# CMU-Perceptual-Computing-Lab/caffe_rtpose

Measured on NVIDIA H100. Metric: frames/sec at 656x368 COCO-18, higher is better.
Workload: dtype f16x2 (2 fp16 planes, 3 wgmma MMAs per MAC, fp32 accumulate)

## Files before the change

### caffe_rtpose_b200/csrc/conv_tc.cu

```cuda
#include <cuda.h>
#include <stdlib.h>
#include <string.h>

#include <algorithm>
#include <atomic>
#include <string>

#include "common.h"
#include "conv_tc.h"
#include "kernels.h"

namespace pe {

struct TcArgs {
    const float* bias;
    __nv_bfloat16* out; int out_pitch, out_coff; long long out_plane;
    float* planar; int planar_C, planar_coff;
    int cout, relu;
    const float* out_scale;
    int ksize, pad, kblocks_per_tap, cin_k;
    int W, H, Wp, Hs;
    long long M;
    int chunk_iters;
    unsigned* range;
};

__device__ __forceinline__ uint32_t smem_u32(const void* p) { return (uint32_t)__cvta_generic_to_shared(p); }

__device__ __forceinline__ void mbar_init(uint64_t* bar, uint32_t count) {
    asm volatile("mbarrier.init.shared::cta.b64 [%0], %1;" ::"r"(smem_u32(bar)), "r"(count));
}
__device__ __forceinline__ void mbar_expect_tx(uint64_t* bar, uint32_t bytes) {
    asm volatile("mbarrier.arrive.expect_tx.shared::cta.b64 _, [%0], %1;" ::"r"(smem_u32(bar)), "r"(bytes) : "memory");
}
__device__ __forceinline__ void mbar_arrive(uint64_t* bar) {
    asm volatile("mbarrier.arrive.shared::cta.b64 _, [%0];" ::"r"(smem_u32(bar)) : "memory");
}
__device__ __forceinline__ void mbar_wait(uint64_t* bar, uint32_t parity) {
    uint32_t done;
    do {
        asm volatile(
            "{\n\t"
            ".reg .pred p;\n\t"
            "mbarrier.try_wait.parity.shared::cta.b64 p, [%1], %2;\n\t"
            "selp.u32 %0, 1, 0, p;\n\t"
            "}" : "=r"(done) : "r"(smem_u32(bar)), "r"(parity) : "memory");
    } while (!done);
}
__device__ __forceinline__ void tma_load_3d(void* dst, const CUtensorMap* map, uint64_t* bar, int c0, int c1, int c2) {
    asm volatile(
        "cp.async.bulk.tensor.3d.shared::cluster.global.tile.mbarrier::complete_tx::bytes [%0], [%1, {%3, %4, %5}], [%2];"
        ::"r"(smem_u32(dst)), "l"(map), "r"(smem_u32(bar)), "r"(c0), "r"(c1), "r"(c2) : "memory");
}

__device__ __forceinline__ void pdl_wait() { asm volatile("griddepcontrol.wait;" ::: "memory"); }
__device__ __forceinline__ void pdl_launch_dependents() { asm volatile("griddepcontrol.launch_dependents;" ::: "memory"); }

__device__ __forceinline__ uint64_t wg_desc(uint32_t saddr) {
    uint64_t d = 0;
    d |= (uint64_t)((saddr >> 4) & 0x3FFF);
    d |= (uint64_t)1 << 16;
    d |= (uint64_t)64 << 32;
    d |= (uint64_t)1 << 62;
    return d;
}
__device__ __forceinline__ void wg_fence() { asm volatile("wgmma.fence.sync.aligned;" ::: "memory"); }
__device__ __forceinline__ void wg_commit() { asm volatile("wgmma.commit_group.sync.aligned;" ::: "memory"); }
__device__ __forceinline__ void wg_wait_all() { asm volatile("wgmma.wait_group.sync.aligned 0;" ::: "memory"); }

template <int N> struct Wgmma;
template <> struct Wgmma<16> {
    template <bool F16> __device__ __forceinline__ static void mma(float* d, uint64_t da, uint64_t db, uint32_t scale_d) {
        if (F16) asm volatile(
            "{\n.reg .pred p;\nsetp.ne.b32 p, %10, 0;\n"
            "wgmma.mma_async.sync.aligned.m64n16k16.f32.f16.f16 {%0,%1,%2,%3,%4,%5,%6,%7}, %8, %9, p, 1, 1, 0, 0;\n}"
            : "+f"(d[0]), "+f"(d[1]), "+f"(d[2]), "+f"(d[3]), "+f"(d[4]), "+f"(d[5]), "+f"(d[6]), "+f"(d[7])
            : "l"(da), "l"(db), "r"(scale_d));
        else asm volatile(
            "{\n.reg .pred p;\nsetp.ne.b32 p, %10, 0;\n"
            "wgmma.mma_async.sync.aligned.m64n16k16.f32.bf16.bf16 {%0,%1,%2,%3,%4,%5,%6,%7}, %8, %9, p, 1, 1, 0, 0;\n}"
            : "+f"(d[0]), "+f"(d[1]), "+f"(d[2]), "+f"(d[3]), "+f"(d[4]), "+f"(d[5]), "+f"(d[6]), "+f"(d[7])
            : "l"(da), "l"(db), "r"(scale_d));
    }
};
template <> struct Wgmma<32> {
    template <bool F16> __device__ __forceinline__ static void mma(float* d, uint64_t da, uint64_t db, uint32_t scale_d) {
        if (F16) asm volatile(
            "{\n.reg .pred p;\nsetp.ne.b32 p, %18, 0;\n"
            "wgmma.mma_async.sync.aligned.m64n32k16.f32.f16.f16 {%0,%1,%2,%3,%4,%5,%6,%7,%8,%9,%10,%11,%12,%13,%14,%15}, %16, %17, p, 1, 1, 0, 0;\n}"
            : "+f"(d[0]), "+f"(d[1]), "+f"(d[2]), "+f"(d[3]), "+f"(d[4]), "+f"(d[5]), "+f"(d[6]), "+f"(d[7]), "+f"(d[8]), "+f"(d[9]), "+f"(d[10]), "+f"(d[11]), "+f"(d[12]), "+f"(d[13]), "+f"(d[14]), "+f"(d[15])
            : "l"(da), "l"(db), "r"(scale_d));
        else asm volatile(
            "{\n.reg .pred p;\nsetp.ne.b32 p, %18, 0;\n"
            "wgmma.mma_async.sync.aligned.m64n32k16.f32.bf16.bf16 {%0,%1,%2,%3,%4,%5,%6,%7,%8,%9,%10,%11,%12,%13,%14,%15}, %16, %17, p, 1, 1, 0, 0;\n}"
            : "+f"(d[0]), "+f"(d[1]), "+f"(d[2]), "+f"(d[3]), "+f"(d[4]), "+f"(d[5]), "+f"(d[6]), "+f"(d[7]), "+f"(d[8]), "+f"(d[9]), "+f"(d[10]), "+f"(d[11]), "+f"(d[12]), "+f"(d[13]), "+f"(d[14]), "+f"(d[15])
            : "l"(da), "l"(db), "r"(scale_d));
    }
};
template <> struct Wgmma<48> {
    template <bool F16> __device__ __forceinline__ static void mma(float* d, uint64_t da, uint64_t db, uint32_t scale_d) {
        if (F16) asm volatile(
            "{\n.reg .pred p;\nsetp.ne.b32 p, %26, 0;\n"
            "wgmma.mma_async.sync.aligned.m64n48k16.f32.f16.f16 {%0,%1,%2,%3,%4,%5,%6,%7,%8,%9,%10,%11,%12,%13,%14,%15,%16,%17,%18,%19,%20,%21,%22,%23}, %24, %25, p, 1, 1, 0, 0;\n}"
            : "+f"(d[0]), "+f"(d[1]), "+f"(d[2]), "+f"(d[3]), "+f"(d[4]), "+f"(d[5]), "+f"(d[6]), "+f"(d[7]), "+f"(d[8]), "+f"(d[9]), "+f"(d[10]), "+f"(d[11]), "+f"(d[12]), "+f"(d[13]), "+f"(d[14]), "+f"(d[15]), "+f"(d[16]), "+f"(d[17]), "+f"(d[18]), "+f"(d[19]), "+f"(d[20]), "+f"(d[21]), "+f"(d[22]), "+f"(d[23])
            : "l"(da), "l"(db), "r"(scale_d));
        else asm volatile(
            "{\n.reg .pred p;\nsetp.ne.b32 p, %26, 0;\n"
            "wgmma.mma_async.sync.aligned.m64n48k16.f32.bf16.bf16 {%0,%1,%2,%3,%4,%5,%6,%7,%8,%9,%10,%11,%12,%13,%14,%15,%16,%17,%18,%19,%20,%21,%22,%23}, %24, %25, p, 1, 1, 0, 0;\n}"
            : "+f"(d[0]), "+f"(d[1]), "+f"(d[2]), "+f"(d[3]), "+f"(d[4]), "+f"(d[5]), "+f"(d[6]), "+f"(d[7]), "+f"(d[8]), "+f"(d[9]), "+f"(d[10]), "+f"(d[11]), "+f"(d[12]), "+f"(d[13]), "+f"(d[14]), "+f"(d[15]), "+f"(d[16]), "+f"(d[17]), "+f"(d[18]), "+f"(d[19]), "+f"(d[20]), "+f"(d[21]), "+f"(d[22]), "+f"(d[23])
            : "l"(da), "l"(db), "r"(scale_d));
    }
};
template <> struct Wgmma<64> {
    template <bool F16> __device__ __forceinline__ static void mma(float* d, uint64_t da, uint64_t db, uint32_t scale_d) {
        if (F16) asm volatile(
            "{\n.reg .pred p;\nsetp.ne.b32 p, %34, 0;\n"
            "wgmma.mma_async.sync.aligned.m64n64k16.f32.f16.f16 {%0,%1,%2,%3,%4,%5,%6,%7,%8,%9,%10,%11,%12,%13,%14,%15,%16,%17,%18,%19,%20,%21,%22,%23,%24,%25,%26,%27,%28,%29,%30,%31}, %32, %33, p, 1, 1, 0, 0;\n}"
            : "+f"(d[0]), "+f"(d[1]), "+f"(d[2]), "+f"(d[3]), "+f"(d[4]), "+f"(d[5]), "+f"(d[6]), "+f"(d[7]), "+f"(d[8]), "+f"(d[9]), "+f"(d[10]), "+f"(d[11]), "+f"(d[12]), "+f"(d[13]), "+f"(d[14]), "+f"(d[15]), "+f"(d[16]), "+f"(d[17]), "+f"(d[18]), "+f"(d[19]), "+f"(d[20]), "+f"(d[21]), "+f"(d[22]), "+f"(d[23]), "+f"(d[24]), "+f"(d[25]), "+f"(d[26]), "+f"(d[27]), "+f"(d[28]), "+f"(d[29]), "+f"(d[30]), "+f"(d[31])
            : "l"(da), "l"(db), "r"(scale_d));
        else asm volatile(
            "{\n.reg .pred p;\nsetp.ne.b32 p, %34, 0;\n"
            "wgmma.mma_async.sync.aligned.m64n64k16.f32.bf16.bf16 {%0,%1,%2,%3,%4,%5,%6,%7,%8,%9,%10,%11,%12,%13,%14,%15,%16,%17,%18,%19,%20,%21,%22,%23,%24,%25,%26,%27,%28,%29,%30,%31}, %32, %33, p, 1, 1, 0, 0;\n}"
            : "+f"(d[0]), "+f"(d[1]), "+f"(d[2]), "+f"(d[3]), "+f"(d[4]), "+f"(d[5]), "+f"(d[6]), "+f"(d[7]), "+f"(d[8]), "+f"(d[9]), "+f"(d[10]), "+f"(d[11]), "+f"(d[12]), "+f"(d[13]), "+f"(d[14]), "+f"(d[15]), "+f"(d[16]), "+f"(d[17]), "+f"(d[18]), "+f"(d[19]), "+f"(d[20]), "+f"(d[21]), "+f"(d[22]), "+f"(d[23]), "+f"(d[24]), "+f"(d[25]), "+f"(d[26]), "+f"(d[27]), "+f"(d[28]), "+f"(d[29]), "+f"(d[30]), "+f"(d[31])
            : "l"(da), "l"(db), "r"(scale_d));
    }
};
template <> struct Wgmma<128> {
    template <bool F16> __device__ __forceinline__ static void mma(float* d, uint64_t da, uint64_t db, uint32_t scale_d) {
        if (F16) asm volatile(
            "{\n.reg .pred p;\nsetp.ne.b32 p, %66, 0;\n"
            "wgmma.mma_async.sync.aligned.m64n128k16.f32.f16.f16 {%0,%1,%2,%3,%4,%5,%6,%7,%8,%9,%10,%11,%12,%13,%14,%15,%16,%17,%18,%19,%20,%21,%22,%23,%24,%25,%26,%27,%28,%29,%30,%31,%32,%33,%34,%35,%36,%37,%38,%39,%40,%41,%42,%43,%44,%45,%46,%47,%48,%49,%50,%51,%52,%53,%54,%55,%56,%57,%58,%59,%60,%61,%62,%63}, %64, %65, p, 1, 1, 0, 0;\n}"
            : "+f"(d[0]), "+f"(d[1]), "+f"(d[2]), "+f"(d[3]), "+f"(d[4]), "+f"(d[5]), "+f"(d[6]), "+f"(d[7]), "+f"(d[8]), "+f"(d[9]), "+f"(d[10]), "+f"(d[11]), "+f"(d[12]), "+f"(d[13]), "+f"(d[14]), "+f"(d[15]), "+f"(d[16]), "+f"(d[17]), "+f"(d[18]), "+f"(d[19]), "+f"(d[20]), "+f"(d[21]), "+f"(d[22]), "+f"(d[23]), "+f"(d[24]), "+f"(d[25]), "+f"(d[26]), "+f"(d[27]), "+f"(d[28]), "+f"(d[29]), "+f"(d[30]), "+f"(d[31]), "+f"(d[32]), "+f"(d[33]), "+f"(d[34]), "+f"(d[35]), "+f"(d[36]), "+f"(d[37]), "+f"(d[38]), "+f"(d[39]), "+f"(d[40]), "+f"(d[41]), "+f"(d[42]), "+f"(d[43]), "+f"(d[44]), "+f"(d[45]), "+f"(d[46]), "+f"(d[47]), "+f"(d[48]), "+f"(d[49]), "+f"(d[50]), "+f"(d[51]), "+f"(d[52]), "+f"(d[53]), "+f"(d[54]), "+f"(d[55]), "+f"(d[56]), "+f"(d[57]), "+f"(d[58]), "+f"(d[59]), "+f"(d[60]), "+f"(d[61]), "+f"(d[62]), "+f"(d[63])
            : "l"(da), "l"(db), "r"(scale_d));
        else asm volatile(
            "{\n.reg .pred p;\nsetp.ne.b32 p, %66, 0;\n"
            "wgmma.mma_async.sync.aligned.m64n128k16.f32.bf16.bf16 {%0,%1,%2,%3,%4,%5,%6,%7,%8,%9,%10,%11,%12,%13,%14,%15,%16,%17,%18,%19,%20,%21,%22,%23,%24,%25,%26,%27,%28,%29,%30,%31,%32,%33,%34,%35,%36,%37,%38,%39,%40,%41,%42,%43,%44,%45,%46,%47,%48,%49,%50,%51,%52,%53,%54,%55,%56,%57,%58,%59,%60,%61,%62,%63}, %64, %65, p, 1, 1, 0, 0;\n}"
            : "+f"(d[0]), "+f"(d[1]), "+f"(d[2]), "+f"(d[3]), "+f"(d[4]), "+f"(d[5]), "+f"(d[6]), "+f"(d[7]), "+f"(d[8]), "+f"(d[9]), "+f"(d[10]), "+f"(d[11]), "+f"(d[12]), "+f"(d[13]), "+f"(d[14]), "+f"(d[15]), "+f"(d[16]), "+f"(d[17]), "+f"(d[18]), "+f"(d[19]), "+f"(d[20]), "+f"(d[21]), "+f"(d[22]), "+f"(d[23]), "+f"(d[24]), "+f"(d[25]), "+f"(d[26]), "+f"(d[27]), "+f"(d[28]), "+f"(d[29]), "+f"(d[30]), "+f"(d[31]), "+f"(d[32]), "+f"(d[33]), "+f"(d[34]), "+f"(d[35]), "+f"(d[36]), "+f"(d[37]), "+f"(d[38]), "+f"(d[39]), "+f"(d[40]), "+f"(d[41]), "+f"(d[42]), "+f"(d[43]), "+f"(d[44]), "+f"(d[45]), "+f"(d[46]), "+f"(d[47]), "+f"(d[48]), "+f"(d[49]), "+f"(d[50]), "+f"(d[51]), "+f"(d[52]), "+f"(d[53]), "+f"(d[54]), "+f"(d[55]), "+f"(d[56]), "+f"(d[57]), "+f"(d[58]), "+f"(d[59]), "+f"(d[60]), "+f"(d[61]), "+f"(d[62]), "+f"(d[63])
            : "l"(da), "l"(db), "r"(scale_d));
    }
};

__device__ __forceinline__ void range_publish(unsigned* range, float m) {
    if (!range) return;
#pragma unroll
    for (int o = 16; o > 0; o >>= 1) m = fmaxf(m, __shfl_xor_sync(0xffffffffu, m, o));
    if ((threadIdx.x & 31) == 0 && m > 0.f) atomicMax(range, __float_as_uint(m));
}

constexpr int TC_BM = 128;
constexpr int TC_BK = 64;
constexpr int TC_WROWS = TC_BM + 8;
constexpr int TC_KMAX = TC_WROWS - TC_BM + 1;
constexpr int TC_THREADS = 384;
constexpr int TC_PRODUCER_REGS = 40, TC_CONSUMER_REGS = 232;
constexpr int TC_SMEM_BUDGET = 220 * 1024;

__host__ __device__ constexpr int tc_window_rows(int ksize) { return ksize == 1 ? TC_BM : TC_WROWS; }

template <int BN, int PLANES> struct TcShape {
    static constexpr int A_BYTES = PLANES * TC_WROWS * 128;
    static constexpr int B_PLANE = BN * 128;
    static constexpr int B_BYTES = PLANES * B_PLANE;
    static constexpr int W_STAGES = 3 * A_BYTES + 6 * B_BYTES <= TC_SMEM_BUDGET ? 3 : 2;
    static constexpr int B_FIT = (TC_SMEM_BUDGET - W_STAGES * A_BYTES) / B_BYTES;
    static constexpr int B_STAGES = B_FIT > 8 ? 8 : B_FIT;
    static constexpr int SMEM = W_STAGES * A_BYTES + B_STAGES * B_BYTES + 1024;
};

template <int BN, int PLANES>
__global__ void __launch_bounds__(TC_THREADS, 1)
conv_wg_kernel(const __grid_constant__ CUtensorMap tmA, const __grid_constant__ CUtensorMap tmB, const TcArgs a) {
    using S = TcShape<BN, PLANES>;
    constexpr int WS = S::W_STAGES, BS = S::B_STAGES;
    constexpr bool F16 = planes_are_fp16(PLANES);
    constexpr int NACC = BN / 2;
    static_assert(S::B_STAGES >= 2, "shared memory holds fewer than two weight tiles");

    extern __shared__ uint8_t smem_raw[];
    uint8_t* smem = (uint8_t*)(((uintptr_t)smem_raw + 1023) & ~(uintptr_t)1023);
    uint8_t* const wring = smem;
    uint8_t* const bring = smem + WS * S::A_BYTES;
    __shared__ __align__(8) uint64_t wfull[WS], wempty[WS], bfull[BS], bempty[BS];
    __shared__ float s_bias[BN];

    const int warp = threadIdx.x >> 5, lane = threadIdx.x & 31;
    const long long m0 = (long long)blockIdx.x * TC_BM;
    const int n0 = blockIdx.y * BN;
    const int ks = a.ksize, taps = ks * ks;
    const int num_k = taps * a.kblocks_per_tap;

    if (threadIdx.x == 0) {
        for (int s = 0; s < WS; s++) { mbar_init(&wfull[s], 1); mbar_init(&wempty[s], 8); }
        for (int s = 0; s < BS; s++) { mbar_init(&bfull[s], 1); mbar_init(&bempty[s], 8); }
        asm volatile("fence.mbarrier_init.release.cluster;" ::: "memory");
        asm volatile("prefetch.tensormap [%0];" ::"l"(&tmA) : "memory");
        asm volatile("prefetch.tensormap [%0];" ::"l"(&tmB) : "memory");
    }
    for (int i = threadIdx.x; i < BN; i += TC_THREADS) s_bias[i] = (n0 + i < a.cout) ? a.bias[n0 + i] : 0.f;
    __syncthreads();
    pdl_launch_dependents();
    pdl_wait();

    if (warp < 4) {
        asm volatile("setmaxnreg.dec.sync.aligned.u32 %0;" ::"n"(TC_PRODUCER_REGS));
        if (threadIdx.x == 0) {
            const uint32_t a_tx = PLANES * tc_window_rows(ks) * 128;
            int wc = 0, bc = 0;
            for (int kb = 0; kb < a.kblocks_per_tap; kb++)
                for (int r = 0; r < ks; r++, wc++) {
                    const int w = wc % WS;
                    mbar_wait(&wempty[w], ((uint32_t)(wc / WS) & 1u) ^ 1u);
                    mbar_expect_tx(&wfull[w], a_tx);
                    const int row0 = (int)(m0 + (long long)(r - a.pad) * a.Wp - a.pad);
                    tma_load_3d(wring + (size_t)w * S::A_BYTES, &tmA, &wfull[w], kb * TC_BK, row0, 0);
                    for (int q = 0; q < ks; q++, bc++) {
                        const int b = bc % BS;
                        mbar_wait(&bempty[b], ((uint32_t)(bc / BS) & 1u) ^ 1u);
                        mbar_expect_tx(&bfull[b], S::B_BYTES);
                        tma_load_3d(bring + (size_t)b * S::B_BYTES, &tmB, &bfull[b], (r * ks + q) * a.cin_k + kb * TC_BK, n0, 0);
                    }
                }
        }
        return;
    }
    asm volatile("setmaxnreg.inc.sync.aligned.u32 %0;" ::"n"(TC_CONSUMER_REGS));

    const int wg = (warp >> 2) - 1;
    float acc_h[NACC], sum_h[NACC], acc_c[NACC];
#pragma unroll
    for (int j = 0; j < NACC; j++) { acc_h[j] = 0.f; sum_h[j] = 0.f; acc_c[j] = 0.f; }
    const int cs = a.chunk_iters;
    const uint32_t a_plane = tc_window_rows(ks) * 128;
    int it = 0, wc = 0;
    for (int kb = 0; kb < a.kblocks_per_tap; kb++)
        for (int r = 0; r < ks; r++, wc++) {
            const int w = wc % WS;
            mbar_wait(&wfull[w], (uint32_t)(wc / WS) & 1u);
            const uint32_t wa = smem_u32(wring + (size_t)w * S::A_BYTES) + (uint32_t)(wg * 64 * 128);
            for (int q = 0; q < ks; q++, it++) {
                const int b = it % BS;
                mbar_wait(&bfull[b], (uint32_t)(it / BS) & 1u);
                const uint32_t sa = wa + (uint32_t)(q * 128);
                const uint32_t sb = smem_u32(bring + (size_t)b * S::B_BYTES);
                const uint32_t h_acc = (it % cs) != 0;
                wg_fence();
#pragma unroll
                for (int k = 0; k < TC_BK / 16; k++) {
                    Wgmma<BN>::template mma<F16>(acc_h, wg_desc(sa + k * 32), wg_desc(sb + k * 32), (k != 0) | h_acc);
                    if constexpr (PLANES > 1) {
#pragma unroll
                        for (int pa = 0; pa < PLANES; pa++)
#pragma unroll
                            for (int pb = 0; pb < PLANES - pa; pb++) {
                                if (pa + pb == 0) continue;
                                const uint32_t first = it == 0 && k == 0 && pa + pb == 1 && pa == 0;
                                Wgmma<BN>::template mma<F16>(acc_c, wg_desc(sa + pa * a_plane + k * 32),
                                                             wg_desc(sb + pb * S::B_PLANE + k * 32), first ? 0u : 1u);
                            }
                    }
                }
                wg_commit();
                wg_wait_all();
                __syncwarp();
                if (lane == 0) mbar_arrive(&bempty[b]);
                if ((it + 1) % cs == 0 || it + 1 == num_k) {
#pragma unroll
                    for (int j = 0; j < NACC; j++) sum_h[j] = __fadd_rn(sum_h[j], acc_h[j]);
                }
            }
            if (lane == 0) mbar_arrive(&wempty[w]);
        }

    const int per_img = a.Hs * a.Wp;
    const int cout8 = (a.cout + 7) & ~7;
    const float out_scale = __ldg(a.out_scale);
    float range_max = 0.f;
#pragma unroll
    for (int hr = 0; hr < 2; hr++) {
        const long long m = m0 + wg * 64 + (warp & 3) * 16 + (lane >> 2) + hr * 8;
        bool valid = m < a.M;
        int n = 0, y = 0, x = 0;
        if (valid) {
            n = (int)(m / per_img);
            const int rem = (int)(m % per_img);
            y = rem / a.Wp; x = rem % a.Wp;
            valid = (x < a.W) && (y < a.H);
        }
        if (!valid) continue;
#pragma unroll
        for (int g = 0; g < BN / 8; g++) {
            const int c = g * 8 + (lane & 3) * 2, j = g * 4 + hr * 2;
            const int co = n0 + c;
            float v[2];
#pragma unroll
            for (int e = 0; e < 2; e++) {
                float t = PLANES > 1 ? __fadd_rn(sum_h[j + e], acc_c[j + e]) : sum_h[j + e];
                t = __fmaf_rn(t, out_scale, s_bias[c + e]);
                if (a.relu) t = fmaxf(t, 0.f);
                v[e] = t;
                if (co + e < a.cout) range_max = fmaxf(range_max, fabsf(t));
            }
            if (a.planar) {
#pragma unroll
                for (int e = 0; e < 2; e++)
                    if (co + e < a.cout) a.planar[(((size_t)n * a.planar_C + a.planar_coff + co + e) * a.H + y) * a.W + x] = v[e];
            } else if (co < cout8) {
                __nv_bfloat16* orow = a.out + (size_t)m * a.out_pitch + a.out_coff + co;
#pragma unroll
                for (int p = 0; p < PLANES; p++) *(uint32_t*)(orow + (size_t)p * a.out_plane) = split_pair<F16>(v[0], v[1]);
            }
        }
    }
    range_publish(a.range, range_max);
}

typedef CUresult (*EncodeTiledFn)(CUtensorMap*, CUtensorMapDataType, cuuint32_t, void*, const cuuint64_t*, const cuuint64_t*,
                                  const cuuint32_t*, const cuuint32_t*, CUtensorMapInterleave, CUtensorMapSwizzle,
                                  CUtensorMapL2promotion, CUtensorMapFloatOOBfill);
static EncodeTiledFn get_encode() {
    static EncodeTiledFn fn = nullptr;
    if (!fn) {
        void* p = nullptr;
        cudaDriverEntryPointQueryResult qr;
        if (cudaGetDriverEntryPoint("cuTensorMapEncodeTiled", &p, cudaEnableDefault, &qr) == cudaSuccess && qr == cudaDriverEntryPointSuccess)
            fn = (EncodeTiledFn)p;
    }
    return fn;
}

int tc_cout_pad(int cout) {
    if (cout >= 128) return (cout + 127) / 128 * 128;
    if (cout > 48) return 64;
    if (cout > 32) return 48;
    if (cout > 16) return 32;
    return 16;
}
static int tc_bn(int cout_pad, int planes) { return std::min(cout_pad, planes == 3 ? 64 : 128); }

static int env_int(const char* name, int dflt) {
    const char* v = getenv(name);
    return v ? atoi(v) : dflt;
}

template <int BN, int PLANES>
static int launch_inst(const TcLayer& l, const TcArgs& a, dim3 grid, cudaStream_t st, int bmap) {
    auto kern = conv_wg_kernel<BN, PLANES>;
    constexpr int smem = TcShape<BN, PLANES>::SMEM;
    int dev = 0;
    cudaGetDevice(&dev);
    static std::atomic<unsigned long long> attr_done{0};
    if (!(attr_done.load(std::memory_order_acquire) >> (dev & 63) & 1ull)) {
        if (cudaFuncSetAttribute(kern, cudaFuncAttributeMaxDynamicSharedMemorySize, smem) != cudaSuccess) return -1;
        attr_done.fetch_or(1ull << (dev & 63), std::memory_order_release);
    }
    cudaLaunchConfig_t cfg = {};
    cfg.gridDim = grid; cfg.blockDim = dim3(TC_THREADS, 1, 1); cfg.dynamicSmemBytes = (size_t)smem; cfg.stream = st;
    cudaLaunchAttribute at[1];
    at[0].id = cudaLaunchAttributeProgrammaticStreamSerialization;
    at[0].val.programmaticStreamSerializationAllowed = 1;
    cfg.attrs = at; cfg.numAttrs = 1;
    const CUtensorMap* maps = (const CUtensorMap*)l.maps;
    return cudaLaunchKernelEx(&cfg, kern, maps[0], maps[bmap], a) == cudaSuccess ? 1 : -1;
}

template <int BN>
static int launch_bn(const TcLayer& l, const TcArgs& a, dim3 grid, cudaStream_t st, int bmap) {
    switch (l.d.planes) {
        case 1: return launch_inst<BN, 1>(l, a, grid, st, bmap);
        case 2: return launch_inst<BN, 2>(l, a, grid, st, bmap);
        default: if constexpr (BN <= 64) return launch_inst<BN, 3>(l, a, grid, st, bmap); else break;
    }
    return -1;
}

static int encode(EncodeTiledFn enc, CUtensorMap* map, const void* base, cuuint64_t d0, cuuint64_t d1, cuuint64_t d2, cuuint64_t s1,
                  cuuint64_t s2, cuuint32_t b1, cuuint32_t b2, CUtensorMapL2promotion l2) {
    cuuint64_t dims[3] = {d0, d1, d2};
    cuuint64_t strides[2] = {s1, s2};
    cuuint32_t box[3] = {(cuuint32_t)TC_BK, b1, b2};
    cuuint32_t es[3] = {1, 1, 1};
    return (int)enc(map, CU_TENSOR_MAP_DATA_TYPE_BFLOAT16, 3, (void*)base, dims, strides, box, es, CU_TENSOR_MAP_INTERLEAVE_NONE,
                    CU_TENSOR_MAP_SWIZZLE_128B, l2, CU_TENSOR_MAP_FLOAT_OOB_FILL_NONE);
}

int tc_layer_create(const TcLayerDesc& d, TcLayer& out, std::string& err) {
    EncodeTiledFn enc = get_encode();
    if (!enc) { err = "cuTensorMapEncodeTiled unavailable"; return -1; }
    if (d.in_cused % TC_BK) { err = "input channels not a multiple of 64"; return -1; }
    if (d.planes < 1 || d.planes > 3) { err = "1 to 3 planes"; return -1; }
    if (d.ksize < 1 || d.ksize > TC_KMAX) { err = "filter size above " + std::to_string(TC_KMAX) + " (A window rows)"; return -1; }
    out.d = d;
    out.bn = tc_bn(d.cout_pad, d.planes);
    CUtensorMap* maps = nullptr;
    if (posix_memalign((void**)&maps, 64, 3 * sizeof(CUtensorMap))) { err = "alloc"; return -1; }
    memset(maps, 0, 3 * sizeof(CUtensorMap));
    const cuuint64_t K = (cuuint64_t)d.ksize * d.ksize * d.in_cused;
    const cuuint64_t P = (cuuint64_t)d.planes;
    int r = encode(enc, &maps[0], d.in, d.in_cused, d.geo.M, P, (cuuint64_t)d.in_pitch * 2, (cuuint64_t)d.in_plane * 2,
                   tc_window_rows(d.ksize), d.planes,
                   CU_TENSOR_MAP_L2_PROMOTION_L2_128B);
    if (!r) r = encode(enc, &maps[1], d.w, K, d.cout_pad, P, K * 2, K * 2 * d.cout_pad, out.bn, d.planes, CU_TENSOR_MAP_L2_PROMOTION_L2_256B);
    if (!r && out.bn >= 64) r = encode(enc, &maps[2], d.w, K, d.cout_pad, P, K * 2, K * 2 * d.cout_pad, out.bn / 2, d.planes, CU_TENSOR_MAP_L2_PROMOTION_L2_256B);
    if (r) { err = "cuTensorMapEncodeTiled failed: " + std::to_string(r); free(maps); return -1; }
    out.maps = maps;
    return 0;
}

void tc_layer_destroy(TcLayer& l) {
    if (l.maps) free(l.maps);
    l.maps = nullptr;
}

int tc_layer_launch(const TcLayer& l, int nimg, cudaStream_t st, int share) {
    const TcLayerDesc& d = l.d;
    TcArgs a;
    a.bias = d.bias;
    a.out = (__nv_bfloat16*)d.out; a.out_pitch = d.out_pitch; a.out_coff = d.out_coff; a.out_plane = d.out_plane;
    a.planar = d.planar; a.planar_C = d.planar_C; a.planar_coff = d.planar_coff;
    a.cout = d.cout; a.relu = d.relu; a.out_scale = d.out_scale; a.range = d.range;
    a.ksize = d.ksize; a.pad = d.pad; a.kblocks_per_tap = d.in_cused / TC_BK; a.cin_k = d.in_cused;
    a.W = d.geo.W; a.H = d.geo.H; a.Wp = d.geo.Wp; a.Hs = d.geo.Hs;
    a.M = (long long)nimg * d.geo.Hs * d.geo.Wp;
    const int nk = d.ksize * d.ksize * a.kblocks_per_tap;
    a.chunk_iters = d.planes >= 2 ? (d.ksize >= 7 ? 7 : (d.ksize >= 3 ? 6 : 4)) : nk;
    static int nsm = 0;
    if (!nsm) { int dev = 0; cudaGetDevice(&dev); cudaDeviceGetAttribute(&nsm, cudaDevAttrMultiProcessorCount, dev); }
    const long long mt = (a.M + TC_BM - 1) / TC_BM;
    const long long sms = std::max(1, nsm / (share < 1 ? 1 : share));
    static const int narrow_env = env_int("PE_TC_NARROW", 1);
    int bn = l.bn, bmap = 1;
    if (narrow_env && l.bn >= 64) {
        const double sfull = (double)std::min<long long>(mt * (d.cout_pad / l.bn), sms) * 1.00;
        const double shalf = (double)std::min<long long>(mt * (d.cout_pad / (l.bn / 2)), sms) * 0.80;
        if (shalf > sfull) { bn = l.bn / 2; bmap = 2; }
    }
    const dim3 grid((unsigned)mt, (unsigned)(d.cout_pad / bn), 1);
    switch (bn) {
        case 128: return launch_bn<128>(l, a, grid, st, bmap);
        case 64: return launch_bn<64>(l, a, grid, st, bmap);
        case 48: return launch_bn<48>(l, a, grid, st, bmap);
        case 32: return launch_bn<32>(l, a, grid, st, bmap);
        default: return launch_bn<16>(l, a, grid, st, bmap);
    }
}

}
```

Baseline: 306.0.

## Multicast weight tiles across 2-CTA clusters and tile M per image

Launches the conv kernel in clusters of two CTAs along M. Each CTA loads half of the shared weight tile and multicasts it to both, and consumers release the weight stage in both CTAs' empty barriers. The aim is to halve the L2 traffic for weight tiles. M tiles are also now indexed per image so that tiles covering only padding rows are skipped. The cost is cluster barrier synchronisation, a final drain wait, smaller TMA boxes, and CTA pairs that must be co-scheduled, which can hurt occupancy.

Measured after the change: 316.5 (median of 6 runs). +3.4%, better.

```diff
diff --git a/caffe_rtpose_b200/csrc/conv_tc.cu b/caffe_rtpose_b200/csrc/conv_tc.cu
--- a/caffe_rtpose_b200/csrc/conv_tc.cu
+++ b/caffe_rtpose_b200/csrc/conv_tc.cu
@@ -21,6 +21,7 @@
     int ksize, pad, kblocks_per_tap, cin_k;
     int W, H, Wp, Hs;
     long long M;
+    int tiles_img;
     int chunk_iters;
     unsigned* range;
 };
@@ -52,6 +53,28 @@
         "cp.async.bulk.tensor.3d.shared::cluster.global.tile.mbarrier::complete_tx::bytes [%0], [%1, {%3, %4, %5}], [%2];"
         ::"r"(smem_u32(dst)), "l"(map), "r"(smem_u32(bar)), "r"(c0), "r"(c1), "r"(c2) : "memory");
 }
+__device__ __forceinline__ void tma_load_3d_mc(void* dst, const CUtensorMap* map, uint64_t* bar, int c0, int c1, int c2, uint16_t mask) {
+    asm volatile(
+        "cp.async.bulk.tensor.3d.shared::cluster.global.tile.mbarrier::complete_tx::bytes.multicast::cluster [%0], [%1, {%3, %4, %5}], [%2], %6;"
+        ::"r"(smem_u32(dst)), "l"(map), "r"(smem_u32(bar)), "r"(c0), "r"(c1), "r"(c2), "h"(mask) : "memory");
+}
+
+__device__ __forceinline__ uint32_t cluster_ctarank() {
+    uint32_t r;
+    asm volatile("mov.u32 %0, %%cluster_ctarank;" : "=r"(r));
+    return r;
+}
+__device__ __forceinline__ void cluster_sync() {
+    asm volatile("barrier.cluster.arrive.release.aligned;\n\tbarrier.cluster.wait.acquire.aligned;" ::: "memory");
+}
+__device__ __forceinline__ void mbar_arrive_cluster(uint64_t* bar, uint32_t rank) {
+    asm volatile(
+        "{\n\t"
+        ".reg .b32 ra;\n\t"
+        "mapa.shared::cluster.u32 ra, %0, %1;\n\t"
+        "mbarrier.arrive.shared::cluster.b64 _, [ra];\n\t"
+        "}" ::"r"(smem_u32(bar)), "r"(rank) : "memory");
+}
 
 __device__ __forceinline__ void pdl_wait() { asm volatile("griddepcontrol.wait;" ::: "memory"); }
 __device__ __forceinline__ void pdl_launch_dependents() { asm volatile("griddepcontrol.launch_dependents;" ::: "memory"); }
@@ -155,7 +178,12 @@
 constexpr int TC_PRODUCER_REGS = 40, TC_CONSUMER_REGS = 232;
 constexpr int TC_SMEM_BUDGET = 220 * 1024;
 
+constexpr int TC_CLUSTER = 2;
+
 __host__ __device__ constexpr int tc_window_rows(int ksize) { return ksize == 1 ? TC_BM : TC_WROWS; }
+
+__host__ __device__ constexpr int tc_gcd(int a, int b) { return b ? tc_gcd(b, a % b) : a; }
+__host__ __device__ constexpr int tc_wbox_rows(int bn, int planes) { return tc_gcd(planes * bn / TC_CLUSTER, bn); }
 
 template <int BN, int PLANES> struct TcShape {
     static constexpr int A_BYTES = PLANES * TC_WROWS * 128;
@@ -175,6 +203,8 @@
     constexpr bool F16 = planes_are_fp16(PLANES);
     constexpr int NACC = BN / 2;
     static_assert(S::B_STAGES >= 2, "shared memory holds fewer than two weight tiles");
+    constexpr int WBOX = tc_wbox_rows(BN, PLANES), WSHARE = PLANES * BN / TC_CLUSTER;
+    static_assert(WSHARE * TC_CLUSTER == PLANES * BN && WBOX % 8 == 0, "weight tile does not split into whole swizzle atoms");
 
     extern __shared__ uint8_t smem_raw[];
     uint8_t* smem = (uint8_t*)(((uintptr_t)smem_raw + 1023) & ~(uintptr_t)1023);
@@ -184,20 +214,21 @@
     __shared__ float s_bias[BN];
 
     const int warp = threadIdx.x >> 5, lane = threadIdx.x & 31;
-    const long long m0 = (long long)blockIdx.x * TC_BM;
+    const int img = blockIdx.x / a.tiles_img;
+    const long long m0 = (long long)img * a.Hs * a.Wp + (long long)(blockIdx.x % a.tiles_img) * TC_BM;
     const int n0 = blockIdx.y * BN;
     const int ks = a.ksize, taps = ks * ks;
     const int num_k = taps * a.kblocks_per_tap;
 
     if (threadIdx.x == 0) {
         for (int s = 0; s < WS; s++) { mbar_init(&wfull[s], 1); mbar_init(&wempty[s], 8); }
-        for (int s = 0; s < BS; s++) { mbar_init(&bfull[s], 1); mbar_init(&bempty[s], 8); }
+        for (int s = 0; s < BS; s++) { mbar_init(&bfull[s], 1); mbar_init(&bempty[s], 8 * TC_CLUSTER); }
         asm volatile("fence.mbarrier_init.release.cluster;" ::: "memory");
         asm volatile("prefetch.tensormap [%0];" ::"l"(&tmA) : "memory");
         asm volatile("prefetch.tensormap [%0];" ::"l"(&tmB) : "memory");
     }
     for (int i = threadIdx.x; i < BN; i += TC_THREADS) s_bias[i] = (n0 + i < a.cout) ? a.bias[n0 + i] : 0.f;
-    __syncthreads();
+    cluster_sync();
     pdl_launch_dependents();
     pdl_wait();
 
@@ -205,6 +236,7 @@
         asm volatile("setmaxnreg.dec.sync.aligned.u32 %0;" ::"n"(TC_PRODUCER_REGS));
         if (threadIdx.x == 0) {
             const uint32_t a_tx = PLANES * tc_window_rows(ks) * 128;
+            const int f0 = (int)cluster_ctarank() * WSHARE;
             int wc = 0, bc = 0;
             for (int kb = 0; kb < a.kblocks_per_tap; kb++)
                 for (int r = 0; r < ks; r++, wc++) {
@@ -217,9 +249,13 @@
                         const int b = bc % BS;
                         mbar_wait(&bempty[b], ((uint32_t)(bc / BS) & 1u) ^ 1u);
                         mbar_expect_tx(&bfull[b], S::B_BYTES);
-                        tma_load_3d(bring + (size_t)b * S::B_BYTES, &tmB, &bfull[b], (r * ks + q) * a.cin_k + kb * TC_BK, n0, 0);
+#pragma unroll
+                        for (int f = f0; f < f0 + WSHARE; f += WBOX)
+                            tma_load_3d_mc(bring + (size_t)b * S::B_BYTES + (size_t)f * 128, &tmB, &bfull[b],
+                                           (r * ks + q) * a.cin_k + kb * TC_BK, n0 + f % BN, f / BN, (uint16_t)((1u << TC_CLUSTER) - 1));
                     }
                 }
+            for (int i = 0; i < BS; i++, bc++) mbar_wait(&bempty[bc % BS], ((uint32_t)(bc / BS) & 1u) ^ 1u);
         }
         return;
     }
@@ -262,7 +298,7 @@
                 wg_commit();
                 wg_wait_all();
                 __syncwarp();
-                if (lane == 0) mbar_arrive(&bempty[b]);
+                if (lane < TC_CLUSTER) mbar_arrive_cluster(&bempty[b], lane);
                 if ((it + 1) % cs == 0 || it + 1 == num_k) {
 #pragma unroll
                     for (int j = 0; j < NACC; j++) sum_h[j] = __fadd_rn(sum_h[j], acc_h[j]);
@@ -278,15 +314,9 @@
 #pragma unroll
     for (int hr = 0; hr < 2; hr++) {
         const long long m = m0 + wg * 64 + (warp & 3) * 16 + (lane >> 2) + hr * 8;
-        bool valid = m < a.M;
-        int n = 0, y = 0, x = 0;
-        if (valid) {
-            n = (int)(m / per_img);
-            const int rem = (int)(m % per_img);
-            y = rem / a.Wp; x = rem % a.Wp;
-            valid = (x < a.W) && (y < a.H);
-        }
-        if (!valid) continue;
+        const int n = (int)(m / per_img), rem = (int)(m % per_img);
+        const int y = rem / a.Wp, x = rem % a.Wp;
+        if (m >= a.M || n != img || x >= a.W || y >= a.H) continue;
 #pragma unroll
         for (int g = 0; g < BN / 8; g++) {
             const int c = g * 8 + (lane & 3) * 2, j = g * 4 + hr * 2;
@@ -355,10 +385,12 @@
     }
     cudaLaunchConfig_t cfg = {};
     cfg.gridDim = grid; cfg.blockDim = dim3(TC_THREADS, 1, 1); cfg.dynamicSmemBytes = (size_t)smem; cfg.stream = st;
-    cudaLaunchAttribute at[1];
+    cudaLaunchAttribute at[2];
     at[0].id = cudaLaunchAttributeProgrammaticStreamSerialization;
     at[0].val.programmaticStreamSerializationAllowed = 1;
-    cfg.attrs = at; cfg.numAttrs = 1;
+    at[1].id = cudaLaunchAttributeClusterDimension;
+    at[1].val.clusterDim.x = TC_CLUSTER; at[1].val.clusterDim.y = 1; at[1].val.clusterDim.z = 1;
+    cfg.attrs = at; cfg.numAttrs = 2;
     const CUtensorMap* maps = (const CUtensorMap*)l.maps;
     return cudaLaunchKernelEx(&cfg, kern, maps[0], maps[bmap], a) == cudaSuccess ? 1 : -1;
 }
@@ -399,8 +431,10 @@
     int r = encode(enc, &maps[0], d.in, d.in_cused, d.geo.M, P, (cuuint64_t)d.in_pitch * 2, (cuuint64_t)d.in_plane * 2,
                    tc_window_rows(d.ksize), d.planes,
                    CU_TENSOR_MAP_L2_PROMOTION_L2_128B);
-    if (!r) r = encode(enc, &maps[1], d.w, K, d.cout_pad, P, K * 2, K * 2 * d.cout_pad, out.bn, d.planes, CU_TENSOR_MAP_L2_PROMOTION_L2_256B);
-    if (!r && out.bn >= 64) r = encode(enc, &maps[2], d.w, K, d.cout_pad, P, K * 2, K * 2 * d.cout_pad, out.bn / 2, d.planes, CU_TENSOR_MAP_L2_PROMOTION_L2_256B);
+    if (!r) r = encode(enc, &maps[1], d.w, K, d.cout_pad, P, K * 2, K * 2 * d.cout_pad, tc_wbox_rows(out.bn, d.planes), 1,
+                       CU_TENSOR_MAP_L2_PROMOTION_L2_256B);
+    if (!r && out.bn >= 64) r = encode(enc, &maps[2], d.w, K, d.cout_pad, P, K * 2, K * 2 * d.cout_pad, tc_wbox_rows(out.bn / 2, d.planes), 1,
+                                       CU_TENSOR_MAP_L2_PROMOTION_L2_256B);
     if (r) { err = "cuTensorMapEncodeTiled failed: " + std::to_string(r); free(maps); return -1; }
     out.maps = maps;
     return 0;
@@ -434,7 +468,9 @@
         const double shalf = (double)std::min<long long>(mt * (d.cout_pad / (l.bn / 2)), sms) * 0.80;
         if (shalf > sfull) { bn = l.bn / 2; bmap = 2; }
     }
-    const dim3 grid((unsigned)mt, (unsigned)(d.cout_pad / bn), 1);
+    a.tiles_img = ((d.geo.H - 1) * d.geo.Wp + d.geo.W + TC_BM - 1) / TC_BM;
+    const long long tiles = ((long long)nimg * a.tiles_img + TC_CLUSTER - 1) / TC_CLUSTER * TC_CLUSTER;
+    const dim3 grid((unsigned)tiles, (unsigned)(d.cout_pad / bn), 1);
     switch (bn) {
         case 128: return launch_bn<128>(l, a, grid, st, bmap);
         case 64: return launch_bn<64>(l, a, grid, st, bmap);
```
